# YuejiangDong/PPEA-Depth

Measured on AMD Instinct MI355X. Metric: training img/s at 640x192 RepLKNet-31B, higher is better.
Workload: dtype bf16; 1 GPU; RepLKNet-31B Stage-1 640x192, 12 frame triplets/GPU, process_batch + backward + grad all-reduce + Adam; global_batch=12, per_gpu_batch=12, parallelism=dp1, use_checkpoint=BN-stat replay, no recompute (288 GB HBM), launch=whole step captured in one hipGraph

## Files before the change

include/ppea_depth.h:

```cpp
#ifndef PPEA_DEPTH_H
#define PPEA_DEPTH_H

#include <stdint.h>

#ifdef __cplusplus
extern "C" {
#endif

#define PPEA_ERR_UNSUPPORTED (-1)
#define PPEA_ERR_ARG (-2)

int ppea_abi_version(void);

int ppea_timestamp(void* slot, void* stream);

int ppea_dwconv_lk_fwd_f32(const float* x, const float* w_big, const float* w_small,
                           float* y_big, float* y_small,
                           int N, int C, int H, int W, int K, int KS, void* stream);
int ppea_dwconv_lk_fwd_bf16(const uint16_t* x, const float* w_big, const float* w_small,
                            uint16_t* y_big, uint16_t* y_small,
                            int N, int C, int H, int W, int K, int KS, void* stream);

int ppea_dwconv_lk_bwd_data_f32(const float* dy_big, const float* dy_small,
                                const float* w_big, const float* w_small, float* dx,
// ... 23 lines not shown
int ppea_dwconv3x3_fwd_bf16(const void* x, const float* w, void* y, int N, int C, int H, int W, int stride, void* stream);
int ppea_dwconv3x3_bwd_data_f32(const void* dy, const float* w, void* dx, int N, int C, int H, int W, int stride, void* stream);
int ppea_dwconv3x3_bwd_data_bf16(const void* dy, const float* w, void* dx, int N, int C, int H, int W, int stride, void* stream);

int ppea_dwconv_lk_bwd_filter_f32(const float* x, const float* dy, float* dw,
                                  int N, int C, int H, int W, int K, void* stream);

int ppea_pwconv_bf16(const void* A, const void* X, const float* bias, void* Y, int B, int M, int K, int HW,
                     void* stream);

int ppea_pwconv_stats_partials(int B, int M, int K, int HW);
int ppea_pwconv_stats_bf16(const void* A, const void* X, const float* bias, void* Y, float* stats, int B, int M, int K,
                           int HW, void* stream);
int ppea_bn_finalize_sums_f32(const float* partial, int P, int C, long count, float eps, float momentum, float* mean,
                              float* var, float* invstd, float* running_mean, float* running_var, void* stream);
int ppea_pwconv_ex_bf16(const void* A, const void* X, const void* bias, int bias_bf16, int epi, const void* aux,
                        void* Y, void* Y2, int B, int M, int K, int HW, int a_transposed, void* stream);
int ppea_dwconv_lk_fwd_bias_act_bf16p(const uint16_t* x, const void* packed, const float* bias, int relu, uint16_t* y, int N,
                                      int C, int H, int W, int K, void* stream);
int ppea_dwconv_lk_fwd_bias_act_f32(const void* x, const float* w, const float* bias, int relu, void* y, int N, int C, int H,
                                    int W, int K, void* stream);
int ppea_dwconv_lk_fwd_bias_act_bf16(const void* x, const float* w, const float* bias, int relu, void* y, int N, int C, int H,
                                     int W, int K, void* stream);
int ppea_dwconv3x3_fwd_affine_f32(const void* x, const float* w, const float* s, const float* o, int relu, void* y, int N, int C,
                                  int H, int W, int stride, void* stream);
int ppea_dwconv3x3_fwd_affine_bf16(const void* x, const float* w, const float* s, const float* o, int relu, void* y, int N, int C,
                                   int H, int W, int stride, void* stream);
int ppea_pwconv_infer_bf16(const void* A, const void* X, const float* s, const float* o, int act, const void* r1,
                           const void* r2, float r2_scale, const float* s2, const float* o2, void* Y, void* Y2, int B, int M,
                           int K, int HW, void* stream);
// ... 272 lines not shown
```

ppea-depth_amd/csrc/bn_common.h:

```cpp
#pragma once
#include "common.h"

namespace {

constexpr int TPB = 256;
constexpr int V = 8;
constexpr int CH_VECS = 8;
constexpr long CHANNEL_ELEMS = 16384;

template <typename T> __device__ __forceinline__ void ld8(const T* p, float (&o)[V]);
template <> __device__ __forceinline__ void ld8<float>(const float* p, float (&o)[V]) {
    const float4 a = reinterpret_cast<const float4*>(p)[0], b = reinterpret_cast<const float4*>(p)[1];
    o[0] = a.x; o[1] = a.y; o[2] = a.z; o[3] = a.w; o[4] = b.x; o[5] = b.y; o[6] = b.z; o[7] = b.w;
}
template <> __device__ __forceinline__ void ld8<uint16_t>(const uint16_t* p, float (&o)[V]) {
    const uint4 a = *reinterpret_cast<const uint4*>(p);
    const uint32_t w[4] = {a.x, a.y, a.z, a.w};
#pragma unroll
    for (int k = 0; k < 4; ++k) {
        o[2 * k] = __uint_as_float(w[k] << 16);
        o[2 * k + 1] = __uint_as_float(w[k] & 0xffff0000u);
    }
}
template <typename T> __device__ __forceinline__ void st8(T* p, const float (&v)[V]);
// ... 45 lines not shown
}
template <typename T>
__device__ __forceinline__ float act_fwd(float u, int act) {
    if (act == 1) return fmaxf(u, 0.f);
    if (act == 2) {
        if constexpr (sizeof(T) == 2) {
            float e;
            return 0.5f * u * (1.f + erf_fast(u * 0.70710678118654752f, e));
        } else {
            return 0.5f * u * (1.f + erff(u * 0.70710678118654752f));
        }
    }
    return u;
}
template <typename T>
__device__ __forceinline__ float act_bwd(float u, int act) {
    if (act == 1) return u > 0.f ? 1.f : 0.f;
    if (act == 2) {
        if constexpr (sizeof(T) == 2) {
            float e;
            const float cdf = 0.5f * (1.f + erf_fast(u * 0.70710678118654752f, e));
            return cdf + u * (0.39894228040143268f * e);
        } else {
            const float cdf = 0.5f * (1.f + erff(u * 0.70710678118654752f));
            const float pdf = 0.39894228040143268f * expf(-0.5f * u * u);
            return cdf + u * pdf;
        }
    }
    return 1.f;
}
// ... 10 lines not shown
```

ppea-depth_amd/csrc/bn_fused.hip:

```cpp
#include "bn_common.h"
#include <cstdlib>

namespace {

template <typename T>
__global__ __launch_bounds__(TPB) void bn_stats(const T* __restrict__ z, float* __restrict__ partial, int N, int C,
                                                int HW) {
    __shared__ float red[4];
    const int n = blockIdx.x / C, c = blockIdx.x - n * C;
    const T* p = z + (long)blockIdx.x * HW;
    const int hv = ((HW % V) == 0) ? HW : 0;
    float s = 0.f;
    for (int i = threadIdx.x * V; i < hv; i += TPB * V) {
        float x[V];
        ld8<T>(p + i, x);
#pragma unroll
        for (int k = 0; k < V; ++k) s += x[k];
    }
    for (int i = hv + threadIdx.x; i < HW; i += TPB) s += ld_f32<T>(p + i);
    const float mean = block_sum(s, red) / (float)HW;
    float m2 = 0.f;
    for (int i = threadIdx.x * V; i < hv; i += TPB * V) {
        float x[V];
        ld8<T>(p + i, x);
// ... 28 lines not shown
    const float cnt = (float)N * (float)HW;
    const float var = m2 / cnt;
    mean_out[c] = mean;
    var_out[c] = var;
    invstd_out[c] = rsqrtf(var + eps);
    if (running_mean != nullptr) {
        const float unbiased = m2 / fmaxf(cnt - 1.f, 1.f);
        running_mean[c] = (1.f - momentum) * running_mean[c] + momentum * mean;
        running_var[c] = (1.f - momentum) * running_var[c] + momentum * unbiased;
    }
}

__global__ __launch_bounds__(256) void bn_finalize_sums(const float* __restrict__ partial, int P, int C, float count,
                                                        float eps, float momentum, float* __restrict__ mean_out,
                                                        float* __restrict__ var_out, float* __restrict__ invstd_out,
                                                        float* __restrict__ running_mean, float* __restrict__ running_var) {
    const int lane = threadIdx.x & 63, c = blockIdx.x * 4 + (threadIdx.x >> 6);
    if (c >= C) return;
    const float2* p = reinterpret_cast<const float2*>(partial) + (long)c * P;
    double s = 0.0, q = 0.0;
#pragma unroll 8
    for (int i = lane; i < P; i += 64) {
        const float2 v = p[i];
        s += (double)v.x; q += (double)v.y;
    }
#pragma unroll
    for (int o = 32; o > 0; o >>= 1) { s += __shfl_xor(s, o, WAVE); q += __shfl_xor(q, o, WAVE); }
    if (lane == 0) {
        const double mean = s / (double)count;
        double var = q / (double)count - mean * mean;
        var = var > 0.0 ? var : 0.0;
        mean_out[c] = (float)mean;
        var_out[c] = (float)var;
        invstd_out[c] = rsqrtf((float)var + eps);
        if (running_mean != nullptr) {
            const float unbiased = (float)(var * (double)count / fmax((double)count - 1.0, 1.0));
            running_mean[c] = (1.f - momentum) * running_mean[c] + momentum * (float)mean;
            running_var[c] = (1.f - momentum) * running_var[c] + momentum * unbiased;
        }
    }
}

__global__ void bn_finalize_packed(const float* __restrict__ partial, int N, int C, int HW,
                                   float* __restrict__ packed) {
    const int c = blockIdx.x * blockDim.x + threadIdx.x;
    if (c == 0) packed[2 * C] = (float)N * (float)HW;
    if (c >= C) return;
    const float* p = partial + (long)c * N * 2;
    float mean = 0.f;
// ... 476 lines not shown
        }
    }
    const float a1 = p.gamma1[c] * is1, o1 = p.beta1[c] - mu1 * a1;
#pragma unroll
    for (int u = 0; u < NV; ++u) {
        const int j = threadIdx.x + u * TPB;
        if (j >= total) break;
        const int n = j / hv, i = j - n * hv;
        const long off = ((long)n * C + c) * HW + i * V;
        const float m = (mask != nullptr) ? mask[n] : 1.f;
        float e1[V], e2[V], o[V];
        if (r1 != nullptr) ld8<T>(r1 + off, e1);
        if (r2 != nullptr) ld8<T>(r2 + off, e2);
#pragma unroll
        for (int k = 0; k < V; ++k) {
            float v = act_fwd<T>(a1 * x1[u][k] + o1, act) * m;
            if (r1 != nullptr) v += e1[k];
            if (r2 != nullptr) v += r2_scale * e2[k];
            o[k] = v;
        }
        st8<T>(y + off, o);
    }
}

template <typename T, bool TWO, int NV>
__global__ __launch_bounds__(TPB) void bn_bwd_channel(const T* __restrict__ dy, const T* __restrict__ dyb, const T* __restrict__ z1,
                                                      const T* __restrict__ z2, Branch b1, Branch b2,
                                                      const float* __restrict__ mask, float inv_count,
                                                      const T* __restrict__ acc, T* __restrict__ dz1,
                                                      T* __restrict__ dz2, float* __restrict__ sums, int act, int N,
                                                      int C, int HW) {
// ... 259 lines not shown
    } else {
        plane = i / HW;
        n = (int)(plane / C); c = (int)(plane - (long)n * C);
    }
    const float a1 = b1.gamma[c] * b1.invstd[c], o1 = b1.beta[c] - b1.mean[c] * a1;
    float a2 = 0.f, o2 = 0.f;
    if (z2 != nullptr) { a2 = b2.gamma[c] * b2.invstd[c]; o2 = b2.beta[c] - b2.mean[c] * a2; }
    const float m = (mask != nullptr) ? mask[n] : 1.f;
    float x1[V], x2[V], q1[V], q2[V], o[V];
    ld8<T>(z1 + i, x1);
    if (z2 != nullptr) ld8<T>(z2 + i, x2);
    if (r1 != nullptr) ld8<T>(r1 + i, q1);
    if (r2 != nullptr) ld8<T>(r2 + i, q2);
#pragma unroll
    for (int k = 0; k < V; ++k) {
        float u = a1 * x1[k] + o1;
        if (z2 != nullptr) u += a2 * x2[k] + o2;
        float v = act_fwd<T>(u, act) * m;
        if (r1 != nullptr) v += q1[k];
        if (r2 != nullptr) v += r2_scale * q2[k];
        o[k] = v;
    }
    st8<T>(y + i, o);
}

template <typename T>
__global__ __launch_bounds__(TPB) void bn_bwd_apply_flat(const T* __restrict__ dy, const T* __restrict__ z1,
                                                         const T* __restrict__ z2, Branch b1, Branch b2,
                                                         const float* __restrict__ mask,
                                                         const float* __restrict__ sums, float inv_count,
                                                         const T* __restrict__ acc, T* __restrict__ dz1,
                                                         T* __restrict__ dz2, float* __restrict__ dgb, float gscale,
                                                         int act, int C, int HW, long total8) {
// ... 302 lines not shown
}

int ppea_bn_stats_f32(const void* z, float* partial, int N, int C, int HW, void* stream) {
    return stats_impl<float>(z, partial, N, C, HW, stream);
}
int ppea_bn_stats_bf16(const void* z, float* partial, int N, int C, int HW, void* stream) {
    return stats_impl<uint16_t>(z, partial, N, C, HW, stream);
}
int ppea_bn_finalize_sums_f32(const float* partial, int P, int C, long count, float eps, float momentum, float* mean,
                              float* var, float* invstd, float* running_mean, float* running_var, void* stream) {
    if (P <= 0 || C <= 0 || count <= 0) return PPEA_ERR_ARG;
    hipLaunchKernelGGL(bn_finalize_sums, dim3((C + 3) / 4), dim3(256), 0, (hipStream_t)stream, partial, P, C, (float)count,
                       eps, momentum, mean, var, invstd, running_mean, running_var);
    return launch_status();
}
int ppea_bn_finalize_f32(const float* partial, int N, int C, int HW, float eps, float momentum, float* mean,
                         float* var, float* invstd, float* running_mean, float* running_var, void* stream) {
    if (N <= 0 || C <= 0 || HW <= 0) return PPEA_ERR_UNSUPPORTED;
    hipLaunchKernelGGL(bn_finalize, dim3((C + 63) / 64), dim3(64), 0, (hipStream_t)stream, partial, N, C, HW, eps,
                       momentum, mean, var, invstd, running_mean, running_var);
    return launch_status();
}
int ppea_bn_stats_final_f32(const void* z, int N, int C, int HW, float eps, float momentum, float* mean, float* var,
                            float* invstd, float* running_mean, float* running_var, void* stream) {
    return stats_final_impl<float>(z, N, C, HW, eps, momentum, mean, var, invstd, running_mean, running_var, stream);
}
int ppea_bn_stats_final_bf16(const void* z, int N, int C, int HW, float eps, float momentum, float* mean, float* var,
                             float* invstd, float* running_mean, float* running_var, void* stream) {
    return stats_final_impl<uint16_t>(z, N, C, HW, eps, momentum, mean, var, invstd, running_mean, running_var, stream);
}
// ... 81 lines not shown
```

ppea-depth_amd/csrc/common.h:

```cpp
#pragma once
#include <hip/hip_runtime.h>
#include <stdint.h>

#define PPEA_ABI_VERSION 17
#define PPEA_ERR_UNSUPPORTED (-1)
#define PPEA_ERR_ARG (-2)
#define WAVE 64

__device__ __forceinline__ float bf16_to_f32(uint16_t v) {
    return __uint_as_float(((uint32_t)v) << 16);
}
__device__ __forceinline__ uint16_t f32_to_bf16(float f) {
    uint32_t u = __float_as_uint(f);
    if ((u & 0x7fffffffu) > 0x7f800000u) return (uint16_t)((u >> 16) | 0x40u);
    u += 0x7fffu + ((u >> 16) & 1u);
    return (uint16_t)(u >> 16);
}

template <typename T> __device__ __forceinline__ float ld_f32(const T* p);
template <> __device__ __forceinline__ float ld_f32<float>(const float* p) { return *p; }
template <> __device__ __forceinline__ float ld_f32<uint16_t>(const uint16_t* p) { return bf16_to_f32(*p); }
template <typename T> __device__ __forceinline__ void st_f32(T* p, float v);
template <> __device__ __forceinline__ void st_f32<float>(float* p, float v) { *p = v; }
template <> __device__ __forceinline__ void st_f32<uint16_t>(uint16_t* p, float v) { *p = f32_to_bf16(v); }
// ... 9 lines not shown
```

ppea-depth_amd/csrc/pwconv.hip:

```cpp
#include "common.h"
#include <cstdlib>
#include <cstring>

namespace {

typedef __attribute__((ext_vector_type(8))) __bf16 bf16x8;
typedef __attribute__((ext_vector_type(4))) float f32x4;
typedef __attribute__((ext_vector_type(4))) short s16x4;
typedef __attribute__((address_space(3))) s16x4* lds_s16x4_ptr;

constexpr int BN = 128;
constexpr int B_STRIDE = 256;
constexpr int a_stride(int bk) { return bk == 32 ? 96 : 160; }

__device__ __forceinline__ int b_swz(int row) { return 4 * (row & 3) + 16 * ((row >> 3) & 1); }

__device__ __forceinline__ float bf2f(uint16_t v) { return __builtin_bit_cast(float, (uint32_t)v << 16); }
__device__ __forceinline__ uint16_t f2bf(float v) { return __builtin_bit_cast(uint16_t, (__bf16)v); }
__device__ __forceinline__ float gelu_f(float x) { return 0.5f * x * (1.f + erff(x * 0.70710678118654752f)); }
__device__ __forceinline__ float dgelu_f(float x) {
    return 0.5f * (1.f + erff(x * 0.70710678118654752f)) + x * 0.3989422804014327f * __expf(-0.5f * x * x);
}

template <int BM, int WM, int WN, int EPI, bool TA, int BK>
// ... 175 lines not shown
}

constexpr int NSTAGE = 3;

struct PwInfer {
    const float* s; const float* o; const uint16_t* r1; const uint16_t* r2; float r2_scale;
    const float* s2; const float* o2; int act;
};
template <int EPI> struct PwExtra {};
template <> struct PwExtra<5> { PwInfer v; };

template <int BK> __device__ __forceinline__ int a_swz16(int row) {
    return BK == 64 ? ((row >> 1) & 7) : (2 * ((row >> 2) & 1));
}

template <int BM, int BK, int EPI, bool TA = false>
__global__ __launch_bounds__(256) void pwconv2_kernel(const uint16_t* __restrict__ A, const uint16_t* __restrict__ X,
                                                      const void* __restrict__ bias, int bias_bf16,
                                                      const uint16_t* __restrict__ aux, uint16_t* __restrict__ Y,
                                                      uint16_t* __restrict__ Y2, int M, int K, int HW, int nb, int mtiles,
                                                      int total, PwExtra<EPI> ex = {}) {
    constexpr int WM = BM >= 64 ? 2 : 1, WN = 4 / WM;
    constexpr int TM = BM / WM, TN = BN / WN, MT = TM / 16, NT = TN / 16;
    static_assert(!TA || BM == 128, "the transposed-A tile reuses the X tile's 256-byte-row layout");
    constexpr int ARB = BK * 2;
    constexpr int A_BYTES = BM * ARB, X_BYTES = BK * B_STRIDE, STAGE = A_BYTES + X_BYTES;
    constexpr int A_INS = A_BYTES / 1024 / 4, X_INS = X_BYTES / 1024 / 4;
    static_assert(A_BYTES % 4096 == 0 && X_BYTES % 4096 == 0, "every wave issues the same number of loads per stage");
    constexpr int LPS = A_INS + X_INS, KH = BK / 32;
    extern __shared__ __attribute__((aligned(16))) uint8_t lds[];

    const int id = blockIdx.x, xcd = id & 7, q8 = total >> 3, r8 = total & 7;
    const int L = (xcd < r8 ? xcd * (q8 + 1) : r8 * (q8 + 1) + (xcd - r8) * q8) + (id >> 3);
    const int mt_i = L % mtiles, pt = L / mtiles;
    const int n = pt / nb, p0 = (pt - n * nb) * BN, m0 = mt_i * BM;

// ... 49 lines not shown
    const int g = lane >> 4, li = lane & 15, q = li >> 2, pp = li & 3;
    const int b_rowi = 8 * g + q, b_s = b_swz(b_rowi);
    int a_off[MT][KH];
#pragma unroll
    for (int i = 0; i < MT; ++i)
#pragma unroll
        for (int h = 0; h < KH; ++h) {
            const int row = wm * TM + 16 * i + li;
            a_off[i][h] = row * ARB + 16 * ((4 * h + g) ^ a_swz16<BK>(row));
        }
    const int x_off = A_BYTES + b_rowi * B_STRIDE;

    const int nk = K / BK;
    issue(0, 0);
    if (nk > 1) issue(1, 1);
    int cur = 0;
    for (int kt = 0; kt < nk; ++kt) {
        if (kt + 1 < nk) asm volatile("s_waitcnt vmcnt(%0)" ::"n"(LPS) : "memory");
        else asm volatile("s_waitcnt vmcnt(0)" ::: "memory");
        __builtin_amdgcn_s_barrier();
        if (kt + 2 < nk) issue(kt + 2, cur >= 1 ? cur - 1 : NSTAGE - 1);
        const uint8_t* buf = lds + cur * STAGE;
#pragma unroll
        for (int h = 0; h < KH; ++h) {
            bf16x8 af[MT], bfr[NT];
#pragma unroll
            for (int i = 0; i < MT; ++i) {
                if constexpr (TA) {
                    const int chunk = (((wm * TM + 16 * i) >> 2) + pp) ^ b_s;
                    const uint8_t* ap = buf + b_rowi * B_STRIDE + h * 32 * B_STRIDE + (chunk << 3);
                    const s16x4 lo = __builtin_amdgcn_ds_read_tr16_b64_v4i16((lds_s16x4_ptr)(ap));
                    const s16x4 hi = __builtin_amdgcn_ds_read_tr16_b64_v4i16((lds_s16x4_ptr)(ap + 4 * B_STRIDE));
                    typedef __attribute__((ext_vector_type(8))) short s16x8a;
                    const s16x8a both = {lo[0], lo[1], lo[2], lo[3], hi[0], hi[1], hi[2], hi[3]};
// ... 126 lines not shown
    c.v2 = 0;
    if (!ta && !(v2env != nullptr && v2env[0] == '0' && v2env[1] == 0)) {
        int bm, bk;
        if (M >= 128 && blocks128 >= 256) { bm = 128; bk = 32; }
        else if (M > 32 && blocks64 >= 256) { bm = 64; bk = (K >= 512 && K % 64 == 0) ? 64 : 32; }
        else if (K % 64 == 0) { bm = 32; bk = 64; }
        else { bm = 64; bk = 32; }
        if (v2env != nullptr && strchr(v2env, ',') != nullptr) { bm = atoi(v2env); bk = atoi(strchr(v2env, ',') + 1); }
        if (bm == 32 && bk == 32) bk = 64;
        if ((bm == 128 || bm == 64 || bm == 32) && (bk == 64 || bk == 32) && K % bk == 0) { c.v2 = 1; c.bm = bm; c.bk = bk; }
    }
    c.wn = c.bm == 32 ? 4 : 2;
    return c;
}

template <int BM, int BK, int EPI, bool TA = false>
int launch_pw2_t(const void* A, const void* X, const void* bias, int bias_bf16, const void* aux, void* Y, void* Y2, int B,
                 int M, int K, int HW, hipStream_t st, PwExtra<EPI> ex = {}) {
    constexpr int smem = NSTAGE * (BM * BK * 2 + BK * B_STRIDE);
    static bool ready = false;
    auto kern = pwconv2_kernel<BM, BK, EPI, TA>;
    if (!ready) {
        hipError_t e = hipFuncSetAttribute(reinterpret_cast<const void*>(kern), hipFuncAttributeMaxDynamicSharedMemorySize, smem);
        if (e != hipSuccess) return (int)e;
        ready = true;
    }
    const int nb = (HW + BN - 1) / BN, mtiles = (M + BM - 1) / BM;
    const long total = (long)nb * mtiles * B;
    if (total > 0x7fffffffL) return PPEA_ERR_UNSUPPORTED;
    hipLaunchKernelGGL(kern, dim3((unsigned)total), dim3(256), smem, st, (const uint16_t*)A, (const uint16_t*)X, bias, bias_bf16,
                       (const uint16_t*)aux, (uint16_t*)Y, (uint16_t*)Y2, M, K, HW, nb, mtiles, (int)total, ex);
    return launch_status();
}

template <int EPI, bool TA>
int launch_pw(const void* A, const void* X, const void* bias, int bias_bf16, const void* aux, void* Y, void* Y2, int B,
              int M, int K, int HW, hipStream_t st) {
    const PwCfg c = pw_choose(B, M, K, HW, TA);
    if constexpr (!TA) {
        if (c.v2) {
#define PW2(BM_, BK_) return launch_pw2_t<BM_, BK_, EPI>(A, X, bias, bias_bf16, aux, Y, Y2, B, M, K, HW, st)
            if (c.bm == 128) { if (c.bk == 64) PW2(128, 64); else PW2(128, 32); }
            if (c.bm == 64) { if (c.bk == 64) PW2(64, 64); else PW2(64, 32); }
            PW2(32, 64);
#undef PW2
        }
// ... 27 lines not shown
    if (B <= 0 || M <= 0 || K <= 0 || HW <= 0 || (K % 32) != 0 || (HW % 8) != 0 || B > 65535)
        return PPEA_ERR_UNSUPPORTED;
    return launch_pw<0, false>(A, X, bias, 0, nullptr, Y, nullptr, B, M, K, HW, (hipStream_t)stream);
}

int ppea_pwconv_stats_partials(int B, int M, int K, int HW) {
    if (B <= 0 || M <= 0 || K <= 0 || HW <= 0) return 0;
    return B * ((HW + BN - 1) / BN) * pw_choose(B, M, K, HW, false).wn;
}
int ppea_pwconv_stats_bf16(const void* A, const void* X, const float* bias, void* Y, float* stats, int B, int M, int K,
                           int HW, void* stream) {
    if (B <= 0 || M <= 0 || K <= 0 || HW <= 0 || (K % 32) != 0 || (HW % 8) != 0 || B > 65535)
        return PPEA_ERR_UNSUPPORTED;
    if (stats == nullptr) return PPEA_ERR_ARG;
    return launch_pw<4, false>(A, X, bias, 0, nullptr, Y, stats, B, M, K, HW, (hipStream_t)stream);
}

int ppea_pwconv_ex_bf16(const void* A, const void* X, const void* bias, int bias_bf16, int epi, const void* aux,
                        void* Y, void* Y2, int B, int M, int K, int HW, int a_transposed, void* stream) {
    if (B <= 0 || M <= 0 || K <= 0 || HW <= 0 || (K % 32) != 0 || (HW % 8) != 0 || B > 65535)
        return PPEA_ERR_UNSUPPORTED;
    if (a_transposed && (M % 8) != 0) return PPEA_ERR_UNSUPPORTED;
    hipStream_t st = (hipStream_t)stream;
    if (epi == 1 && !Y2) return PPEA_ERR_ARG;
    if (epi == 2 && !aux) return PPEA_ERR_ARG;
    if (a_transposed) {
        switch (epi) {
            case 0: return launch_pw<0, true>(A, X, bias, bias_bf16, nullptr, Y, nullptr, B, M, K, HW, st);
            case 1: return launch_pw<1, true>(A, X, bias, bias_bf16, nullptr, Y, Y2, B, M, K, HW, st);
            case 2: return launch_pw<2, true>(A, X, nullptr, 0, aux, Y, nullptr, B, M, K, HW, st);
// ... 32 lines not shown
```

ppea-depth_amd/ppeadepth/_abi.py:

```python
import ctypes
import os

import torch

_HERE = os.path.dirname(os.path.abspath(__file__))
LIB_PATH = os.path.join(os.path.dirname(_HERE), "libppea_depth.so")

ABI_VERSION = 17

_vp, _i, _l, _f = ctypes.c_void_p, ctypes.c_int, ctypes.c_long, ctypes.c_float

SIGNATURES = {
    "ppea_abi_version": [],
    "ppea_timestamp": [_vp, _vp],
    "ppea_dwconv_lk_fwd_f32": [_vp] * 5 + [_i] * 6 + [_vp],
    "ppea_dwconv_lk_fwd_bf16": [_vp] * 5 + [_i] * 6 + [_vp],
    "ppea_dwconv_lk_bwd_data_f32": [_vp] * 5 + [_i] * 6 + [_vp],
    "ppea_dwconv_lk_bwd_data_bf16": [_vp] * 5 + [_i] * 6 + [_vp],
    "ppea_dwconv_lk_bwd_filter_f32": [_vp] * 3 + [_i] * 5 + [_vp],
    "ppea_dwconv3x3_fwd_f32": [_vp, _vp, _vp, _i, _i, _i, _i, _i, _vp],
    "ppea_dwconv3x3_fwd_bf16": [_vp, _vp, _vp, _i, _i, _i, _i, _i, _vp],
    "ppea_dwconv3x3_bwd_data_f32": [_vp, _vp, _vp, _i, _i, _i, _i, _i, _vp],
    "ppea_dwconv3x3_bwd_data_bf16": [_vp, _vp, _vp, _i, _i, _i, _i, _i, _vp],
    "ppea_dwconv_lk_packed_bytes": [_i, _i],
# ... 111 lines not shown
    "ppea_conv_packed_bytes": [_i] * 5,
    "ppea_conv_pack_weights": [_vp, _i, _vp, _i, _i, _i, _i, _i, _vp],
    "ppea_image_to_nhwc_bf16": [_vp, _vp, _i, _i, _i, _i, _i, _f, _f, _vp],
    "ppea_conv_nhwc_bf16": [_vp, _vp, _vp, _i, _vp] + [_i] * 15 + [_vp],
    "ppea_conv_wgrad_workspace_bytes": [_i] * 8,
    "ppea_conv_wgrad_nhwc_bf16": [_vp, _vp, _vp, _i, _vp] + [_i] * 12 + [_vp],
    "ppea_nhwc_up2cat_fwd_f32": [_vp, _vp, _vp, _i, _i, _i, _i, _i, _vp],
    "ppea_nhwc_up2cat_fwd_bf16": [_vp, _vp, _vp, _i, _i, _i, _i, _i, _vp],
    "ppea_nhwc_up2cat_bwd_f32": [_vp, _vp, _vp, _i, _i, _i, _i, _i, _vp],
    "ppea_nhwc_up2cat_bwd_bf16": [_vp, _vp, _vp, _i, _i, _i, _i, _i, _vp],
    "ppea_dwconv_lk_stats_partials": [_i] * 6,
    "ppea_dwconv_lk_fwd_stats_bf16p": [_vp] * 6 + [_i] * 6 + [_vp],
    "ppea_pwconv_stats_partials": [_i] * 4,
    "ppea_pwconv_stats_bf16": [_vp] * 5 + [_i] * 4 + [_vp],
    "ppea_bn_finalize_sums_f32": [_vp, _i, _i, ctypes.c_long, _f, _f, _vp, _vp, _vp, _vp, _vp, _vp],
    "ppea_conv2d_f32_fwd": [_vp] * 6 + [_i] * 9 + [_vp],
    "ppea_conv2d_f32_dgrad": [_vp] * 5 + [_i] * 11 + [_vp],
    "ppea_conv2d_f32_wgrad_workspace_bytes": [_i] * 7,
    "ppea_conv2d_f32_wgrad": [_vp] * 6 + [_i] * 11 + [_vp],
    "ppea_conv2d_bf16_fwd": [_vp] * 6 + [_i] * 9 + [_vp],
    "ppea_conv2d_bf16_dgrad": [_vp] * 5 + [_i] * 11 + [_vp],
    "ppea_conv2d_bf16_wgrad": [_vp] * 6 + [_i] * 11 + [_vp],
    "ppea_nhwc_maxpool3x3s2_fwd_f32": [_vp, _vp, _vp, _i, _i, _i, _i, _vp],
    "ppea_nhwc_maxpool3x3s2_fwd_bf16": [_vp, _vp, _vp, _i, _i, _i, _i, _vp],
    "ppea_nhwc_maxpool3x3s2_bwd_f32": [_vp, _vp, _vp, _i, _i, _i, _i, _vp],
    "ppea_nhwc_maxpool3x3s2_bwd_bf16": [_vp, _vp, _vp, _i, _i, _i, _i, _vp],
    "ppea_loss_tail_blocks": [_l],
    "ppea_loss_tail_fwd_f32": [_vp] * 10 + [_i] * 4 + [_vp],
    "ppea_loss_tail_bwd_f32": [_vp] * 9 + [_i] * 3 + [_vp],
    "ppea_cost_volume_reduce_f32": [_vp] * 6 + [_i] * 4 + [_vp],
# ... 65 lines not shown
```

ppea-depth_amd/ppeadepth/networks/replknet_adapter.py:

```python
import os
import sys

import torch
import torch.nn as nn
import torch.nn.functional as F

from .. import ops, rng
from ..batchnorm import BatchNorm2d, fused_bn_act, fused_bn_act_next, second_use

FUSE_BN = True
ADAPTER_CHANNELS_LAST = True

use_sync_bn = False


def enable_sync_bn():
    global use_sync_bn
    use_sync_bn = True


def get_bn(channels):
    return BatchNorm2d(channels, sync=use_sync_bn)


# ... 100 lines not shown
    def forward_sums(self, x, always=False):
        from ..batchnorm import _collectives_on
        if (PW_MFMA and BN_SUMS and x.is_cuda and x.dtype == torch.bfloat16 and not self.weight.requires_grad
                and (always or x.shape[0] * x.shape[2] * x.shape[3] > 16384 or _collectives_on())):
            r = ops.pwconv_frozen(x, self.weight, want_sums=True)
            if r is not None:
                return r
        return self.forward(x), None


PW_MFMA = True
DW_SUMS = os.environ.get("PPEA_DW_SUMS", "0") == "1"
DW_BN_FUSE = os.environ.get("PPEA_DW_BN", "1") == "1"
BN_SUMS = os.environ.get("PPEA_BN_SUMS", "1") == "1"
BN_SUMS_FFN = os.environ.get("PPEA_BN_SUMS_FFN", "1") == "1"
ADAPTER_MFMA = True


def get_conv2d(in_channels, out_channels, kernel_size, stride, padding, dilation, groups, bias):
    k = kernel_size if isinstance(kernel_size, int) else kernel_size[0]
    if k == 1 and stride == 1 and padding == 0 and groups == 1 and dilation == 1 and not bias:
        return PointwiseConv(in_channels, out_channels, 1, 1, 0, 1, 1, False)
    if (in_channels == out_channels == groups and k == 3 and stride in (1, 2) and padding == 1 and dilation == 1
            and groups > 1):
        return SmallDW(in_channels, out_channels, 3, stride, 1, 1, groups, bias)
    if (in_channels == out_channels == groups and k > 5 and stride == 1 and padding == k // 2
            and dilation == 1):
        return LargeKernelDW(in_channels, k, bias=bias)
    if groups == 1 and k == 3 and in_channels < 8 and dilation == 1:
        return ImageConv(in_channels, out_channels, 3, stride, padding, dilation, 1, bias)
# ... 190 lines not shown
    def __init__(self, in_channels, internal_channels, out_channels, drop_path, gamma=1.0, adpt_test=0,
                 ratio=0.25):
        super().__init__()
        self.inline_adapter = False
        self.drop_path = DropPath(drop_path) if drop_path > 0.0 else nn.Identity()
        self.preffn_bn = get_bn(in_channels)
        self.pw1 = conv_bn(in_channels, internal_channels, 1, 1, 0, 1)
        self.pw2 = conv_bn(internal_channels, out_channels, 1, 1, 0, 1)
        self.nonlinear = nn.GELU()
        if adpt_test >= 0:
            self.mlp_adapter = Adapter(in_channels, adpt_test, 0.5 if adpt_test == 2 else 0.25)
        self.gamma, self.test_id = gamma, adpt_test

    pre_bn = property(lambda self: self.preffn_bn)

    def forward(self, x, pre_out=None, next_bn=None):
        if FUSE_BN and self.training and x.is_cuda:
            if pre_out is not None:
                out = pre_out
            else:
                out, x = fused_bn_act(x, self.preffn_bn, skip=True)
            adpt, join = None, None
            if self.test_id >= 0:
                if ADAPTER_STREAMS and not self.inline_adapter and torch.cuda.current_stream().cuda_stream not in NO_FORK_ON:
                    adpt, join = _forked_adapter(self.mlp_adapter, second_use(out) if BN_DUP_FORKED else out)
                else:
                    adpt = self.mlp_adapter(second_use(out))
            z1, s1 = _conv_sums(self.pw1.conv, out, BN_SUMS_FFN)
            h = fused_bn_act(z1, self.pw1.bn, act=ops.ACT_GELU, sums=s1)
            z, s2 = _conv_sums(self.pw2.conv, h)
            if join is not None:
                join()
            mask = _drop_mask(self.drop_path, x)
            if next_bn is not None:
                pair = fused_bn_act_next(z, self.pw2.bn, next_bn, mask=mask, r1=x, r2=adpt, r2_scale=self.gamma, sums=s2)
                if pair is not None:
                    return pair
            y = fused_bn_act(z, self.pw2.bn, mask=mask, r1=x, r2=adpt, r2_scale=self.gamma, sums=s2)
            return y if next_bn is None else (y, None)
        assert pre_out is None and next_bn is None
        out = self.preffn_bn(x)
        adpt = self.mlp_adapter(out) if self.test_id >= 0 else None
        out = self.pw2(self.nonlinear(self.pw1(out)))
        y = x + self.drop_path(out)
        return y if adpt is None else y + self.gamma * adpt
# ... 261 lines not shown
```

ppea-depth_amd/ppeadepth/ops.py:

```python
import weakref

import torch

from . import _abi
from ._abi import call, ptr, stream_ptr, try_call

_F32 = torch.float32
_BF16 = torch.bfloat16

PROFILE_DWCONV = None


PROFILE_REPLAY = {}


def _timed(kind, K, fn):
    if PROFILE_DWCONV is None or K != 31:
        return fn()
    PROFILE_REPLAY.setdefault(kind, fn)
    s, e = torch.cuda.Event(enable_timing=True), torch.cuda.Event(enable_timing=True)
    s.record()
    r = fn()
    e.record()
    PROFILE_DWCONV.append((kind, s, e))
# ... 1217 lines not shown
    @staticmethod
    def backward(ctx, dy, _dsums=None):
        return pwconv_raw(ctx.at, dy.contiguous().to(_BF16)), None, None


def pwconv_frozen(x, w, want_sums=False):
    B, K, H, W = x.shape
    if (x.dtype != _BF16 or not x.is_cuda or K % 32 != 0 or w.shape[0] % 32 != 0 or (H * W) % 8 != 0
            or w.requires_grad):
        return None
    if want_sums:
        return _PwConvFrozen.apply(x, w, True)
    return _PwConvFrozen.apply(x, w)


EPI_NONE, EPI_GELU, EPI_DGELU = 0, 1, 2


def _bias_arg(b):
    if b is None:
        return None, 0
    if b.dtype == _BF16:
        return ptr(b, _BF16), 1
    return ptr(b, _F32), 0


def pwconv_ex(a_mat, x, bias=None, epi=EPI_NONE, aux=None, transposed=False):
    B, K, H, W = x.shape
    M = a_mat.shape[1] if transposed else a_mat.shape[0]
    y = torch.empty(B, M, H, W, device=x.device, dtype=_BF16)
# ... 780 lines not shown
```

Baseline: 368.3 img/s.

## Fuse FFN BatchNorm+GELU into the pw2 GEMM operand load

Adds a BN finalize variant that emits a per-channel (scale, offset) table, plus a pwconv2 kernel variant that applies affine+GELU in place on the X tile in LDS before the MFMA loop. The FFN forward uses it to skip materializing the GELU activation h and its separate elementwise kernel. Backward recomputes from z1 via the existing BN-backward kernels. This is gated to layers where the GEMM has at most FFN_BN_TILES M-tiles (default 1), so the transform is not redundantly repeated across many M tiles. It adds ALU work and an extra LDS write and barrier wait inside the GEMM loop.

```diff
diff --git a/include/ppea_depth.h b/include/ppea_depth.h
--- a/include/ppea_depth.h
+++ b/include/ppea_depth.h
@@ -61,6 +61,12 @@
                            int HW, void* stream);
 int ppea_bn_finalize_sums_f32(const float* partial, int P, int C, long count, float eps, float momentum, float* mean,
                               float* var, float* invstd, float* running_mean, float* running_var, void* stream);
+int ppea_bn_finalize_sums_table_f32(const float* partial, int P, int C, long count, float eps, float momentum,
+                                    const float* gamma, const float* beta, float* mean, float* invstd, float* running_mean,
+                                    float* running_var, float* table, void* stream);
+int ppea_pwconv_bnact_supported(int B, int M, int K, int HW);
+int ppea_pwconv_bnact_bf16(const void* A, const void* X, const float* table, void* Y, float* stats, int B, int M, int K,
+                           int HW, void* stream);
 int ppea_pwconv_ex_bf16(const void* A, const void* X, const void* bias, int bias_bf16, int epi, const void* aux,
                         void* Y, void* Y2, int B, int M, int K, int HW, int a_transposed, void* stream);
 int ppea_dwconv_lk_fwd_bias_act_bf16p(const uint16_t* x, const void* packed, const float* bias, int relu, uint16_t* y, int N,
diff --git a/ppea-depth_amd/csrc/bn_common.h b/ppea-depth_amd/csrc/bn_common.h
--- a/ppea-depth_amd/csrc/bn_common.h
+++ b/ppea-depth_amd/csrc/bn_common.h
@@ -83,6 +83,8 @@
     return u;
 }
 template <typename T>
+__device__ __forceinline__ float bn_affine_act(float a, float x, float o, int act) { return act_fwd<T>(a * x + o, act); }
+template <typename T>
 __device__ __forceinline__ float act_bwd(float u, int act) {
     if (act == 1) return u > 0.f ? 1.f : 0.f;
     if (act == 2) {
diff --git a/ppea-depth_amd/csrc/bn_fused.hip b/ppea-depth_amd/csrc/bn_fused.hip
--- a/ppea-depth_amd/csrc/bn_fused.hip
+++ b/ppea-depth_amd/csrc/bn_fused.hip
@@ -66,7 +66,10 @@
 __global__ __launch_bounds__(256) void bn_finalize_sums(const float* __restrict__ partial, int P, int C, float count,
                                                         float eps, float momentum, float* __restrict__ mean_out,
                                                         float* __restrict__ var_out, float* __restrict__ invstd_out,
-                                                        float* __restrict__ running_mean, float* __restrict__ running_var) {
+                                                        float* __restrict__ running_mean, float* __restrict__ running_var,
+                                                        const float* __restrict__ gamma = nullptr,
+                                                        const float* __restrict__ beta = nullptr,
+                                                        float2* __restrict__ table = nullptr) {
     const int lane = threadIdx.x & 63, c = blockIdx.x * 4 + (threadIdx.x >> 6);
     if (c >= C) return;
     const float2* p = reinterpret_cast<const float2*>(partial) + (long)c * P;
@@ -82,9 +85,14 @@
         const double mean = s / (double)count;
         double var = q / (double)count - mean * mean;
         var = var > 0.0 ? var : 0.0;
-        mean_out[c] = (float)mean;
-        var_out[c] = (float)var;
-        invstd_out[c] = rsqrtf((float)var + eps);
+        const float mu = (float)mean, is = rsqrtf((float)var + eps);
+        mean_out[c] = mu;
+        if (var_out != nullptr) var_out[c] = (float)var;
+        invstd_out[c] = is;
+        if (table != nullptr) {
+            const float a = gamma[c] * is;
+            table[c] = make_float2(a, beta[c] - mu * a);
+        }
         if (running_mean != nullptr) {
             const float unbiased = (float)(var * (double)count / fmax((double)count - 1.0, 1.0));
             running_mean[c] = (1.f - momentum) * running_mean[c] + momentum * (float)mean;
@@ -591,7 +599,7 @@
         if (r2 != nullptr) ld8<T>(r2 + off, e2);
 #pragma unroll
         for (int k = 0; k < V; ++k) {
-            float v = act_fwd<T>(a1 * x1[u][k] + o1, act) * m;
+            float v = bn_affine_act<T>(a1, x1[u][k], o1, act) * m;
             if (r1 != nullptr) v += e1[k];
             if (r2 != nullptr) v += r2_scale * e2[k];
             o[k] = v;
@@ -881,9 +889,7 @@
     if (r2 != nullptr) ld8<T>(r2 + i, q2);
 #pragma unroll
     for (int k = 0; k < V; ++k) {
-        float u = a1 * x1[k] + o1;
-        if (z2 != nullptr) u += a2 * x2[k] + o2;
-        float v = act_fwd<T>(u, act) * m;
+        float v = (z2 == nullptr ? bn_affine_act<T>(a1, x1[k], o1, act) : act_fwd<T>(a1 * x1[k] + o1 + (a2 * x2[k] + o2), act)) * m;
         if (r1 != nullptr) v += q1[k];
         if (r2 != nullptr) v += r2_scale * q2[k];
         o[k] = v;
@@ -1216,6 +1222,15 @@
                        eps, momentum, mean, var, invstd, running_mean, running_var);
     return launch_status();
 }
+int ppea_bn_finalize_sums_table_f32(const float* partial, int P, int C, long count, float eps, float momentum,
+                                    const float* gamma, const float* beta, float* mean, float* invstd, float* running_mean,
+                                    float* running_var, float* table, void* stream) {
+    if (P <= 0 || C <= 0 || count <= 0 || gamma == nullptr || beta == nullptr || table == nullptr) return PPEA_ERR_ARG;
+    hipLaunchKernelGGL(bn_finalize_sums, dim3((C + 3) / 4), dim3(256), 0, (hipStream_t)stream, partial, P, C, (float)count,
+                       eps, momentum, mean, (float*)nullptr, invstd, running_mean, running_var, gamma, beta,
+                       reinterpret_cast<float2*>(table));
+    return launch_status();
+}
 int ppea_bn_finalize_f32(const float* partial, int N, int C, int HW, float eps, float momentum, float* mean,
                          float* var, float* invstd, float* running_mean, float* running_var, void* stream) {
     if (N <= 0 || C <= 0 || HW <= 0) return PPEA_ERR_UNSUPPORTED;
diff --git a/ppea-depth_amd/csrc/common.h b/ppea-depth_amd/csrc/common.h
--- a/ppea-depth_amd/csrc/common.h
+++ b/ppea-depth_amd/csrc/common.h
@@ -2,7 +2,7 @@
 #include <hip/hip_runtime.h>
 #include <stdint.h>
 
-#define PPEA_ABI_VERSION 17
+#define PPEA_ABI_VERSION 18
 #define PPEA_ERR_UNSUPPORTED (-1)
 #define PPEA_ERR_ARG (-2)
 #define WAVE 64
diff --git a/ppea-depth_amd/csrc/pwconv.hip b/ppea-depth_amd/csrc/pwconv.hip
--- a/ppea-depth_amd/csrc/pwconv.hip
+++ b/ppea-depth_amd/csrc/pwconv.hip
@@ -1,4 +1,4 @@
-#include "common.h"
+#include "bn_common.h"
 #include <cstdlib>
 #include <cstring>
 
@@ -213,12 +213,13 @@
     return BK == 64 ? ((row >> 1) & 7) : (2 * ((row >> 2) & 1));
 }
 
-template <int BM, int BK, int EPI, bool TA = false>
+template <int BM, int BK, int EPI, bool TA = false, bool XF = false>
 __global__ __launch_bounds__(256) void pwconv2_kernel(const uint16_t* __restrict__ A, const uint16_t* __restrict__ X,
                                                       const void* __restrict__ bias, int bias_bf16,
                                                       const uint16_t* __restrict__ aux, uint16_t* __restrict__ Y,
                                                       uint16_t* __restrict__ Y2, int M, int K, int HW, int nb, int mtiles,
-                                                      int total, PwExtra<EPI> ex = {}) {
+                                                      int total, const float2* __restrict__ xtab, PwExtra<EPI> ex = {}) {
+    static_assert(!XF || !TA, "the transform is on the activation operand of the forward GEMM");
     constexpr int WM = BM >= 64 ? 2 : 1, WN = 4 / WM;
     constexpr int TM = BM / WM, TN = BN / WN, MT = TM / 16, NT = TN / 16;
     static_assert(!TA || BM == 128, "the transposed-A tile reuses the X tile's 256-byte-row layout");
@@ -298,10 +299,43 @@
     const int nk = K / BK;
     issue(0, 0);
     if (nk > 1) issue(1, 1);
+    float tab_a[XF ? X_INS : 1], tab_o[XF ? X_INS : 1];
+    const int lg = lane >> 4;
+    auto load_tab = [&](int kt) {
+#pragma unroll
+        for (int c = 0; c < X_INS; ++c) {
+            typedef __attribute__((ext_vector_type(8))) float f32x8;
+            const f32x8 e = *reinterpret_cast<const f32x8*>(xtab + (kt * BK + 4 * (c * 4 + wave)));
+            const float a01 = lg & 1 ? e[2] : e[0], a23 = lg & 1 ? e[6] : e[4];
+            const float o01 = lg & 1 ? e[3] : e[1], o23 = lg & 1 ? e[7] : e[5];
+            tab_a[c] = lg & 2 ? a23 : a01;
+            tab_o[c] = lg & 2 ? o23 : o01;
+        }
+    };
+    if constexpr (XF) load_tab(0);
     int cur = 0;
     for (int kt = 0; kt < nk; ++kt) {
         if (kt + 1 < nk) asm volatile("s_waitcnt vmcnt(%0)" ::"n"(LPS) : "memory");
         else asm volatile("s_waitcnt vmcnt(0)" ::: "memory");
+        if constexpr (XF) {
+            uint8_t* xs = lds + cur * STAGE + A_BYTES + wave * 1024 + lane * 16;
+#pragma unroll
+            for (int c = 0; c < X_INS; ++c) {
+                const float2 ao = make_float2(tab_a[c], tab_o[c]);
+                const uint4 v = *reinterpret_cast<const uint4*>(xs + c * 4096);
+                const uint32_t w[4] = {v.x, v.y, v.z, v.w};
+                uint32_t o[4];
+#pragma unroll
+                for (int r = 0; r < 4; ++r) {
+                    const float lo = bn_affine_act<uint16_t>(ao.x, __uint_as_float(w[r] << 16), ao.y, 2);
+                    const float hi = bn_affine_act<uint16_t>(ao.x, __uint_as_float(w[r] & 0xffff0000u), ao.y, 2);
+                    o[r] = (uint32_t)f2bf(lo) | ((uint32_t)f2bf(hi) << 16);
+                }
+                *reinterpret_cast<uint4*>(xs + c * 4096) = make_uint4(o[0], o[1], o[2], o[3]);
+            }
+            if (kt + 1 < nk) load_tab(kt + 1);
+            asm volatile("s_waitcnt lgkmcnt(0)" ::: "memory");
+        }
         __builtin_amdgcn_s_barrier();
         if (kt + 2 < nk) issue(kt + 2, cur >= 1 ? cur - 1 : NSTAGE - 1);
         const uint8_t* buf = lds + cur * STAGE;
@@ -458,12 +492,12 @@
     return c;
 }
 
-template <int BM, int BK, int EPI, bool TA = false>
+template <int BM, int BK, int EPI, bool TA = false, bool XF = false>
 int launch_pw2_t(const void* A, const void* X, const void* bias, int bias_bf16, const void* aux, void* Y, void* Y2, int B,
-                 int M, int K, int HW, hipStream_t st, PwExtra<EPI> ex = {}) {
+                 int M, int K, int HW, hipStream_t st, PwExtra<EPI> ex = {}, const float* xtab = nullptr) {
     constexpr int smem = NSTAGE * (BM * BK * 2 + BK * B_STRIDE);
     static bool ready = false;
-    auto kern = pwconv2_kernel<BM, BK, EPI, TA>;
+    auto kern = pwconv2_kernel<BM, BK, EPI, TA, XF>;
     if (!ready) {
         hipError_t e = hipFuncSetAttribute(reinterpret_cast<const void*>(kern), hipFuncAttributeMaxDynamicSharedMemorySize, smem);
         if (e != hipSuccess) return (int)e;
@@ -473,7 +507,8 @@
     const long total = (long)nb * mtiles * B;
     if (total > 0x7fffffffL) return PPEA_ERR_UNSUPPORTED;
     hipLaunchKernelGGL(kern, dim3((unsigned)total), dim3(256), smem, st, (const uint16_t*)A, (const uint16_t*)X, bias, bias_bf16,
-                       (const uint16_t*)aux, (uint16_t*)Y, (uint16_t*)Y2, M, K, HW, nb, mtiles, (int)total, ex);
+                       (const uint16_t*)aux, (uint16_t*)Y, (uint16_t*)Y2, M, K, HW, nb, mtiles, (int)total,
+                       reinterpret_cast<const float2*>(xtab), ex);
     return launch_status();
 }
 
@@ -531,6 +566,26 @@
         return PPEA_ERR_UNSUPPORTED;
     if (stats == nullptr) return PPEA_ERR_ARG;
     return launch_pw<4, false>(A, X, bias, 0, nullptr, Y, stats, B, M, K, HW, (hipStream_t)stream);
+}
+
+int ppea_pwconv_bnact_supported(int B, int M, int K, int HW) {
+    if (B <= 0 || M <= 0 || K <= 0 || HW <= 0 || (K % 32) != 0 || (HW % 8) != 0 || B > 65535) return 0;
+    const PwCfg c = pw_choose(B, M, K, HW, false);
+    return c.v2 ? (M + c.bm - 1) / c.bm : 0;
+}
+int ppea_pwconv_bnact_bf16(const void* A, const void* X, const float* table, void* Y, float* stats, int B, int M, int K,
+                           int HW, void* stream) {
+    if (!ppea_pwconv_bnact_supported(B, M, K, HW)) return PPEA_ERR_UNSUPPORTED;
+    if (A == nullptr || X == nullptr || table == nullptr || Y == nullptr) return PPEA_ERR_ARG;
+    const PwCfg c = pw_choose(B, M, K, HW, false);
+    hipStream_t st = (hipStream_t)stream;
+#define PW2X(BM_, BK_)                                                                                                      \
+    return stats != nullptr ? launch_pw2_t<BM_, BK_, 4, false, true>(A, X, nullptr, 0, nullptr, Y, stats, B, M, K, HW, st, {}, table) \
+                            : launch_pw2_t<BM_, BK_, 0, false, true>(A, X, nullptr, 0, nullptr, Y, nullptr, B, M, K, HW, st, {}, table)
+    if (c.bm == 128) { if (c.bk == 64) PW2X(128, 64); else PW2X(128, 32); }
+    if (c.bm == 64) { if (c.bk == 64) PW2X(64, 64); else PW2X(64, 32); }
+    PW2X(32, 64);
+#undef PW2X
 }
 
 int ppea_pwconv_ex_bf16(const void* A, const void* X, const void* bias, int bias_bf16, int epi, const void* aux,
diff --git a/ppea-depth_amd/ppeadepth/_abi.py b/ppea-depth_amd/ppeadepth/_abi.py
--- a/ppea-depth_amd/ppeadepth/_abi.py
+++ b/ppea-depth_amd/ppeadepth/_abi.py
@@ -6,7 +6,7 @@
 _HERE = os.path.dirname(os.path.abspath(__file__))
 LIB_PATH = os.path.join(os.path.dirname(_HERE), "libppea_depth.so")
 
-ABI_VERSION = 17
+ABI_VERSION = 18
 
 _vp, _i, _l, _f = ctypes.c_void_p, ctypes.c_int, ctypes.c_long, ctypes.c_float
 
@@ -149,6 +149,9 @@
     "ppea_pwconv_stats_partials": [_i] * 4,
     "ppea_pwconv_stats_bf16": [_vp] * 5 + [_i] * 4 + [_vp],
     "ppea_bn_finalize_sums_f32": [_vp, _i, _i, ctypes.c_long, _f, _f, _vp, _vp, _vp, _vp, _vp, _vp],
+    "ppea_bn_finalize_sums_table_f32": [_vp, _i, _i, ctypes.c_long, _f, _f] + [_vp] * 8,
+    "ppea_pwconv_bnact_supported": [_i] * 4,
+    "ppea_pwconv_bnact_bf16": [_vp] * 5 + [_i] * 4 + [_vp],
     "ppea_conv2d_f32_fwd": [_vp] * 6 + [_i] * 9 + [_vp],
     "ppea_conv2d_f32_dgrad": [_vp] * 5 + [_i] * 11 + [_vp],
     "ppea_conv2d_f32_wgrad_workspace_bytes": [_i] * 7,
diff --git a/ppea-depth_amd/ppeadepth/networks/replknet_adapter.py b/ppea-depth_amd/ppeadepth/networks/replknet_adapter.py
--- a/ppea-depth_amd/ppeadepth/networks/replknet_adapter.py
+++ b/ppea-depth_amd/ppeadepth/networks/replknet_adapter.py
@@ -138,6 +138,8 @@
 DW_BN_FUSE = os.environ.get("PPEA_DW_BN", "1") == "1"
 BN_SUMS = os.environ.get("PPEA_BN_SUMS", "1") == "1"
 BN_SUMS_FFN = os.environ.get("PPEA_BN_SUMS_FFN", "1") == "1"
+FFN_BN_FUSE = os.environ.get("PPEA_FFN_BN", "1")
+FFN_BN_TILES = int(os.environ.get("PPEA_FFN_BN_TILES", "1"))
 ADAPTER_MFMA = True
 
 
@@ -358,6 +360,26 @@
 
     pre_bn = property(lambda self: self.preffn_bn)
 
+    def _pw2_bn_fused(self, z1, s1):
+        from .. import batchnorm as bnm
+        conv, bn = self.pw2.conv, self.pw1.bn
+        if not (FFN_BN_FUSE != "0" and PW_MFMA and s1 is not None and isinstance(conv, PointwiseConv) and bn.training
+                and not (bn.sync and bnm._collectives_on()) and bn.running_mean.dtype == torch.float32
+                and not conv.weight.requires_grad and z1.dtype == torch.bfloat16 and z1.is_cuda):
+            return None
+        tiles = ops.pwconv_bnact_tiles(z1.shape, conv.out_channels)
+        if tiles == 0 or (FFN_BN_FUSE != "all" and tiles > FFN_BN_TILES):
+            return None
+        cnt = z1.numel() // z1.shape[1]
+        z, s2, st = ops.pwconv_bnact(z1, s1, bn, conv.weight, want_sums=BN_SUMS and cnt > 16384)
+        if bnm._ACTIVE_DEFERRED is None:
+            bn.num_batches_tracked += 1
+        else:
+            bnm._ACTIVE_DEFERRED.count(bn)
+            if bn.replay_update and torch.is_grad_enabled():
+                bnm._ACTIVE_DEFERRED.add(bn, st[0], st[1], float(cnt))
+        return z, s2
+
     def forward(self, x, pre_out=None, next_bn=None):
         if FUSE_BN and self.training and x.is_cuda:
             if pre_out is not None:
@@ -371,8 +393,12 @@
                 else:
                     adpt = self.mlp_adapter(second_use(out))
             z1, s1 = _conv_sums(self.pw1.conv, out, BN_SUMS_FFN)
-            h = fused_bn_act(z1, self.pw1.bn, act=ops.ACT_GELU, sums=s1)
-            z, s2 = _conv_sums(self.pw2.conv, h)
+            fused = self._pw2_bn_fused(z1, s1)
+            if fused is not None:
+                z, s2 = fused
+            else:
+                h = fused_bn_act(z1, self.pw1.bn, act=ops.ACT_GELU, sums=s1)
+                z, s2 = _conv_sums(self.pw2.conv, h)
             if join is not None:
                 join()
             mask = _drop_mask(self.drop_path, x)
diff --git a/ppea-depth_amd/ppeadepth/ops.py b/ppea-depth_amd/ppeadepth/ops.py
--- a/ppea-depth_amd/ppeadepth/ops.py
+++ b/ppea-depth_amd/ppeadepth/ops.py
@@ -1255,6 +1255,73 @@
     return _PwConvFrozen.apply(x, w)
 
 
+class _PwConvBnAct(torch.autograd.Function):
+
+    @staticmethod
+    def forward(ctx, z1, sums, gamma, beta, rm, rv, eps, momentum, w2, want_sums):
+        z1 = z1.contiguous()
+        N, K, H, W = z1.shape
+        a, at = _pw_matrices(w2)
+        M = a.shape[0]
+        g, b = gamma.detach().float().contiguous(), beta.detach().float().contiguous()
+        st = torch.empty(2, K, device=z1.device, dtype=_F32)
+        table = torch.empty(K, 2, device=z1.device, dtype=_F32)
+        sums = sums.contiguous()
+        call("ppea_bn_finalize_sums_table_f32", ptr(sums, _F32), int(sums.shape[1]), K, N * H * W, float(eps), float(momentum),
+             ptr(g), ptr(b), ptr(st[0]), ptr(st[1]), ptr(rm), ptr(rv), ptr(table), stream_ptr())
+        y = torch.empty(N, M, H, W, device=z1.device, dtype=_BF16)
+        sums2 = None
+        if want_sums:
+            sums2 = torch.empty(M, _abi.lib.ppea_pwconv_stats_partials(N, M, K, H * W), 2, device=z1.device, dtype=_F32)
+        call("ppea_pwconv_bnact_bf16", ptr(a, _BF16), ptr(z1, _BF16), ptr(table), ptr(y), ptr(sums2), N, M, K, H * W, stream_ptr())
+        ctx.save_for_backward(z1, st, g, b)
+        ctx.at = at
+        ctx.pdt = (gamma.dtype, beta.dtype)
+        ctx.mark_non_differentiable(st)
+        if sums2 is not None:
+            ctx.mark_non_differentiable(sums2)
+        ctx.set_materialize_grads(False)
+        return y, sums2, st
+
+    @staticmethod
+    def backward(ctx, dy, _dsums, _dst):
+        z1, st, g, b = ctx.saved_tensors
+        N, C, H, W = z1.shape
+        HW = H * W
+        dh = pwconv_raw(ctx.at, dy.contiguous().to(_BF16))
+        stats = _stats_array((st[0], st[1], g, b, None, None, None, None))
+        sums = torch.empty(3, C, device=z1.device, dtype=_F32)
+        dz = torch.empty_like(z1)
+        if bn_channel_ok(z1):
+            call("ppea_bn_bwd_channel_bf16", ptr(dh), ptr(z1), None, stats, None, 1.0 / float(N * HW), None, ptr(dz), None,
+                 ptr(sums), ACT_GELU, N, C, HW, stream_ptr())
+        else:
+            if not try_call("ppea_bn_bwd_reduce_final_bf16", ptr(dh), ptr(z1), None, stats, None, ptr(sums), ACT_GELU, N, C,
+                            HW, stream_ptr()):
+                partial = torch.empty(C * N * 3, device=z1.device, dtype=_F32)
+                call("ppea_bn_bwd_reduce_bf16", ptr(dh), ptr(z1), None, stats, None, ptr(partial), ACT_GELU, N, C, HW,
+                     stream_ptr())
+                call("ppea_bn_bwd_finalize_f32", ptr(partial), N, C, ptr(sums), stream_ptr())
+            call("ppea_bn_bwd_apply_bf16", ptr(dh), ptr(z1), None, stats, None, ptr(sums), 1.0 / float(N * HW), ptr(dz), None,
+                 ACT_GELU, N, C, HW, stream_ptr())
+        dg = sums[1].to(ctx.pdt[0]) if ctx.needs_input_grad[2] else None
+        db = sums[0].to(ctx.pdt[1]) if ctx.needs_input_grad[3] else None
+        return dz, None, dg, db, None, None, None, None, None, None
+
+
+def pwconv_bnact_tiles(shape, M):
+    N, K, H, W = shape
+    if K % 32 != 0 or M % 32 != 0 or (H * W) % 8 != 0:
+        return 0
+    return int(_abi.lib.ppea_pwconv_bnact_supported(N, M, K, H * W))
+
+
+def pwconv_bnact(z1, sums, bn, w2, want_sums=False):
+    assert not w2.requires_grad and z1.dtype == _BF16 and pwconv_bnact_tiles(z1.shape, w2.shape[0]) > 0
+    return _PwConvBnAct.apply(z1, sums, bn.weight, bn.bias, bn.running_mean, bn.running_var, bn.eps, bn.momentum, w2,
+                              bool(want_sums))
+
+
 EPI_NONE, EPI_GELU, EPI_DGELU = 0, 1, 2
 
 
```

Result: no change. 371.3 img/s (median of 6 runs) (+0.8%).
